# tylerrleee/mcmc-gpu

Hardware: AMD Instinct MI355X
Metric: chain-steps/sec on 256x256 grid x 1024 chains; accept-rate parity (higher is better)
Workload: dtype f64; 1 GPU; largeScaleChain 256x256 grid, 1024 chains/GPU, fp64, Philox spectral (Matern 0.9125) proposals, blocks 50-80, sigma_mc 5 (BASELINE configs[1]); chains_total=1024, mh_steps_per_bench_step=2048

## Files before the change

mcmc_gpu_amd/csrc/chain_strip_kernel.hip:

```cpp
#include "gsm_internal.h"
#include "device_util.h"
#include "proposal_device.h"
#include "strip_step.h"
#include <math.h>
#include <stdlib.h>
#include <algorithm>
#include <type_traits>

namespace gsm {

using namespace dev;
using strip::kST;
using strip::kSW;
using strip::kNR;

constexpr int kSUPW = 32 / kSW;
constexpr int kSMAXT = 16 / kSW;

static int strip_tile_len(const BlockTable& B) { return (B.max_bh + 2) * (B.max_bw + 2); }
static int strip_main_len(const FusedArgs& a) { return std::max(a.P.lds_main, strip_tile_len(a.T.B)); }
constexpr int kStripAux = 16 + 32 + 16 + kMathTabDoubles + 4 * kT1S + kMask1D;
size_t fused_strip_lds_doubles(const FusedArgs& a) { return (size_t)strip_main_len(a) + kStripAux; }

bool strip_table_ok(const StaticFields& S, const BlockTable& B, int lds_main, int tiles1_max, int tiles2_max) {
  static int on = -1;
  if (on < 0) { const char* v = getenv("GSM_STRIP"); on = v ? atoi(v) : 1; }
  const size_t lds = ((size_t)std::max(lds_main, strip_tile_len(B)) + kStripAux) * sizeof(double);
  return on && S.sA != nullptr && (uint64_t)S.H * S.W * 48u <= (4ull << 20) && B.n_sizes <= 64 && strip::table_ok(B.max_bh, B.max_bw) &&
         B.max_bh <= kT1S && B.max_bw <= kT1S && (B.masks == nullptr || B.mask1d != nullptr) && lds <= 80 * 1024 && 2 * tiles1_max <= kSW * kSUPW && tiles2_max <= kSW * kSMAXT;
}

using step::crec_t;
using step::load_c;

template <typename TS, bool FAST_DIV, bool NOISE>
__global__ __launch_bounds__(kST, 4) void chain_strip_kernel(const FusedArgs fa) {
  typedef step::cptr_t<FusedArgs> cargs_t;
  auto kargs = [] { return step::kargs<FusedArgs>(); };
  extern __shared__ double lds[];
  double* __restrict__ red = lds + fa.work_len;
  double* __restrict__ red2 = red + 16;
  double* __restrict__ carry = red2 + 32;
  double* __restrict__ mtab = red2 + 32 + 16;
  double* __restrict__ t1 = mtab + kMathTabDoubles;
  double* __restrict__ m1 = t1 + 4 * kT1S;

  const int tid = threadIdx.x;
  const int lane = tid & 63;
  const int wave = __builtin_amdgcn_readfirstlane(tid >> 6);
  const int chain = blockIdx.x;
  const int n_steps = fa.T.n_steps;
  const int gH = fa.T.S.H, gW = fa.T.S.W;
  const TS* const p_bed = (const TS*)fa.T.beds + (size_t)chain * (size_t)gH * (size_t)gW;
  const TS* const p_en = (const TS*)fa.T.energy + (size_t)chain * (size_t)gH * (size_t)gW;
  const double2* const p_st = fa.T.S.sA;
  const double two_sigma2 = fa.T.S.two_sigma2, rcp_two_sigma2 = fa.T.S.rcp_two_sigma2;
  const uint32_t n_cells = (uint32_t)gH * (uint32_t)gW;
  const crec_t rec0 = (crec_t)(uintptr_t)(fa.P.scalars + (size_t)chain * fa.P.n_steps);
  const uint64_t seed = NOISE ? 0ull : fa.P.seeds[chain];
  for (int i = tid; i < kMathTabDoubles; i += kST) mtab[i] = fa.P.mathtab[i];
  if (tid < 16) red[tid] = 0.0;
  __syncthreads();

  if (tid == 0) {
    const double h0 = fa.T.loss_sum[2 * chain], l0 = fa.T.loss_sum[2 * chain + 1];
    carry[0] = h0; carry[1] = l0; carry[2] = (h0 + l0) / two_sigma2;
  }
  __syncthreads();
  step::Window prev = {};
  const int64_t noise0 = NOISE ? (int64_t)chain * fa.P.n_steps * fa.noise_stride : 0;
  auto prop_rec = [&](crec_t r) {
    PropScalars q;
    q.scale = r->scale; q.nug = r->nug; q.aa = r->aa; q.m_const = r->m_const; q.m_kappa = r->m_kappa;
    q.bh = r->bh; q.bw = r->bw; q.fy_off = r->fy_off; q.g_off = r->g_off; q.pad = r->pad; q.mask_off = r->mask_off;
    q.m_nc = r->m_nc; q.m_m1 = r->m_m1; q.m_bh = r->m_bh; q.m_bw = r->m_bw;
    return q;
  };

  for (int s = 0; s < n_steps; ++s) {
    int ptid = tid;
    asm volatile("" : "+v"(ptid));
    auto relaunder = [&] { asm volatile("" : "+v"(ptid)); };
    const crec_t rec = rec0 + s;
    const int s_row = rec->row, s_col = rec->col, s_bh = rec->bh, s_bw = rec->bw;

    {
      const cargs_t K = kargs();
      const double* __restrict__ g1 = K->P.tab1d;
      if (tid >= kST - kMask1D) m1[tid - (kST - kMask1D)] = K->P.B.mask1d[rec->si * kMask1D + tid - (kST - kMask1D)];
      if (tid < 2 * s_bh) t1[(tid < s_bh) ? tid : kT1S + tid - s_bh] = g1[rec->t1h_off + tid];
      else if (tid >= 256 && tid < 256 + 2 * s_bw) {
        const int i = ptid - 256;
        const double v = g1[rec->t1w_off + i];
        t1[2 * kT1S + ((i < s_bw) ? i : kT1S + i - s_bw)] = (i < s_bw) ? v : -v;
      }
    }
    {
      const cargs_t K = kargs();
      const ProposeArgs pa = load_c(&K->P);
      const PropScalars q = prop_rec(rec);
      const PropGeom pg = prop_geom(pa, q.bh, q.bw);
      NoiseIn nz{nullptr, nullptr, nullptr};
      if (NOISE) {
        const cargs_t F = K;
        const int64_t o = noise0 + (int64_t)s * F->noise_stride;
        nz.re = F->noise_re + o; nz.im = F->noise_im + o;
      }
      coef_items<kST, NOISE, true>(ptid, pa, q, pg, seed, pa.step0 + s, lds, nz, mtab, pa.parseval ? red2 + 16 : nullptr);
    }
    if (step::halo_touches(step::clip_window(gH, gW, s_row, s_col, s_bh, s_bw), prev)) asm volatile("s_waitcnt vmcnt(0)" ::: "memory");
    asm volatile("s_waitcnt lgkmcnt(0)\n\ts_barrier" ::: "memory");
    const double dc0 = lds[0];
    {
      v4f64 uc[kSUPW], us[kSUPW];
      {
        const cargs_t K = kargs();
        const ProposeArgs pa = load_c(&K->P);
        const PropScalars q = prop_rec(rec);
        dft_stage1<kSW, kSUPW, kTabLds1D>(wave, ptid & 63, pa, q, prop_geom(pa, q.bh, q.bw), lds, t1, uc, us);
      }
      asm volatile("s_waitcnt lgkmcnt(0)\n\ts_barrier" ::: "memory");
      {
        const cargs_t K = kargs();
        const ProposeArgs pa = load_c(&K->P);
        relaunder();
        dft_tt_write<kSW, kSUPW>(wave, ptid & 63, prop_geom(pa, s_bh, s_bw), lds, uc, us);
      }
    }
    asm volatile("s_waitcnt lgkmcnt(0)\n\ts_barrier" ::: "memory");
    {
      const cargs_t K = kargs();
      const ProposeArgs pa = load_c(&K->P);
      const PropScalars q = prop_rec(rec);
      const PropGeom pg = prop_geom(pa, q.bh, q.bw);
      const int bw = q.bw;
      v4f64 fe[kSMAXT], fo[kSMAXT];
      const double mreg[kSMAXT][8] = {};
      relaunder();
      const int ln = ptid & 63;
      dft_stage2<kSW, kSMAXT, kTabLds1D>(wave, ln, pa, q, pg, lds, t1 + 2 * kT1S, fe, fo);
      const double gain = standardise<kSW, kSMAXT>(wave, ln, q, pg, dc0, red2, fe, fo, pa.parseval ? red2 + 16 : nullptr);
      NoiseIn nz{nullptr, nullptr, nullptr};
      if (NOISE) {
        const cargs_t F = K;
        const double* nb = F->noise_nug;
        if (nb) nz.nug = nb + noise0 + (int64_t)s * F->noise_stride;
      }
      const bool with_nugget = NOISE ? (nz.nug != nullptr) : (pa.rf.nugget_max > 0.0);
      emit_field<kSW, kSMAXT, kMaskLds1D>(wave, ln, pa, q, pg, fe, fo, mreg, gain, with_nugget, lds, [bw](int y, int x) { return (y + 1) * (bw + 2) + x + 1; }, m1);
      if (with_nugget) {
        __syncthreads();
        relaunder();
        nugget_pass<kST, NOISE>(ptid, pa, q, pg, seed, pa.step0 + s, nz, lds, [bw](int y, int x) { return (y + 1) * (bw + 2) + x + 1; }, mtab);
      }
    }
    relaunder();
    const step::Window Gw = step::clip_window(gH, gW, s_row, s_col, s_bh, s_bw);
    const strip::Window G = strip::make_window(gH, gW, s_row, s_col, s_bh, s_bw);
    const strip::Cfg cfg = strip::config(G.wh, G.ww);
    const strip::Lane L = strip::lane_setup(ptid & 63, wave, cfg, G, gH, gW);
    const rsrc_t r_bed = make_rsrc(p_bed, n_cells * (uint32_t)sizeof(TS));
    const rsrc_t r_en = make_rsrc(p_en, n_cells * (uint32_t)sizeof(TS));
    const rsrc_t r_st = make_rsrc(p_st, 3u * n_cells * 16u);
    uint32_t upd_bits;
    double acc_old;
    bool guard;
    {
      double vb[kNR + 2], ve[kNR];
      double2 a2[strip::kNA];
      if (G.interior) strip::load_state<TS, true>(L, cfg.n, gW, r_bed, r_en, r_st, vb, ve, a2);
      else strip::load_state<TS, false>(L, cfg.n, gW, r_bed, r_en, r_st, vb, ve, a2);
      asm volatile("s_waitcnt lgkmcnt(0)\n\ts_barrier" ::: "memory");
      const int ts = s_bw + 2;
      auto field = [&](int jj, bool) { return lds[L.tidx + jj * ts]; };
      if (G.interior) strip::phase_a<TS, true>(L, cfg.n, gW, s_bw, r_st, field, lds, vb, ve, a2, upd_bits, acc_old, guard);
      else strip::phase_a<TS, false>(L, cfg.n, gW, s_bw, r_st, field, lds, vb, ve, a2, upd_bits, acc_old, guard);
    }
    asm volatile("s_waitcnt lgkmcnt(0)\n\ts_barrier" ::: "memory");
    double en[kNR], vn[kNR];
    {
      double acc_new;
      const cargs_t K = kargs();
      const step::StepConsts SC{K->T.S.res, K->T.S.rcp_res, K->T.S.two_res, K->T.S.rcp_two_res};
      if (G.interior) strip::phase_d<TS, FAST_DIV, true>(L, cfg.n, gW, s_bw, r_st, n_cells * 16u, SC, lds, en, acc_new);
      else strip::phase_d<TS, FAST_DIV, false>(L, cfg.n, gW, s_bw, r_st, n_cells * 16u, SC, lds, en, acc_new);
      double delta = acc_new - acc_old;
      if (guard) delta = INFINITY;
      const double w_delta = wave64_sum(delta);
      if (lane == 0) red[wave] = w_delta;
    }
    strip::read_candidate(L, cfg.n, s_bw, lds, vn);
    const double s_hi = carry[0], s_lo = carry[1];
    double loss_prev = carry[2];
    asm volatile("s_waitcnt lgkmcnt(0)\n\ts_barrier" ::: "memory");
    const double sd = strip::waves_sum(red, lane);
    double c_hi, c_lo, loss_next;
    const bool acc = step::decide<FAST_DIV>(sd, sd == INFINITY, s_hi, s_lo, two_sigma2, rcp_two_sigma2, loss_prev, rec->u, c_hi, c_lo, loss_next);
    if (acc) {
      if (G.interior) strip::commit<TS, true, false>(L, cfg.n, gW, r_bed, r_en, r_en, vn, en, upd_bits);
      else strip::commit<TS, false, false>(L, cfg.n, gW, r_bed, r_en, r_en, vn, en, upd_bits);
      loss_prev = loss_next;
      if (tid == 0) {
        double n_hi, n_lo;
        two_sum(c_hi, c_lo, n_hi, n_lo);
        carry[0] = n_hi; carry[1] = n_lo; carry[2] = loss_next;
      }
      prev = Gw;
    } else {
      prev = step::Window{};
    }
    if (tid == 0) {
      const cargs_t Ke = kargs();
      const StepArgs a = load_c(&Ke->T);
      step::write_record(a, step::record_index(a, chain, s), loss_prev, acc, s_row, s_col, s_bh, s_bw);
    }
  }
  if (tid == 0) {
    fa.T.loss_sum[2 * chain] = carry[0];
    fa.T.loss_sum[2 * chain + 1] = carry[1];
  }
}

template <typename TS, bool FAST_DIV>
__global__ __launch_bounds__(kST, 4) void step_strip_kernel(const StepArgs a) {
  extern __shared__ double tile[];
  __shared__ double red[16];
  __shared__ int tab[2 * 64];
  const StaticFields& S = a.S;
  const int tid = threadIdx.x;
  const int lane = tid & 63;
  const int wave = __builtin_amdgcn_readfirstlane(tid >> 6);
  const int chain = blockIdx.x;
  const int H = S.H, W = S.W;
  const uint32_t n_cells = (uint32_t)H * (uint32_t)W;
  const size_t plane = (size_t)H * W;
  const rsrc_t r_bed = make_rsrc((const TS*)a.beds + (size_t)chain * plane, n_cells * (uint32_t)sizeof(TS));
  const rsrc_t r_en = make_rsrc((const TS*)a.energy + (size_t)chain * plane, n_cells * (uint32_t)sizeof(TS));
  const rsrc_t r_rs = make_rsrc(a.resampled + (size_t)chain * plane, n_cells * 4u);
  const rsrc_t r_st = make_rsrc(S.sA, 3u * n_cells * 16u);
  const step::StepConsts SC{S.res, S.rcp_res, S.two_res, S.rcp_two_res};

  double s_hi = a.loss_sum[2 * chain], s_lo = a.loss_sum[2 * chain + 1];
  double loss_prev = (s_hi + s_lo) / S.two_sigma2;
  for (int i = tid; i < a.B.n_sizes; i += kST) { tab[2 * i] = a.B.bh[i]; tab[2 * i + 1] = a.B.bw[i]; }
  if (tid < 16) red[tid] = 0.0;
  const int64_t rin0 = (int64_t)chain * a.in_stride;
  step::ReplayRec nxt = step::read_replay(a, rin0);
  __syncthreads();

  for (int s = 0; s < a.n_steps; ++s) {
    const int64_t rin = rin0 + s;
    const int64_t rout = step::record_index(a, chain, s);
    const step::ReplayRec cur = nxt;
    const bool has_next = s + 1 < a.n_steps;
    if (has_next) nxt = step::read_replay(a, rin + 1);
    if (!step::replay_valid(a, cur)) {
      if (tid == 0) step::reject_record(a, rout, loss_prev, cur);
      continue;
    }
    const int bh = tab[2 * cur.si], bw = tab[2 * cur.si + 1];
    const rsrc_t r_f = make_rsrc(a.fields + rin * a.field_stride, (uint32_t)(bh * bw) * 8u);
    const step::Window Gw = step::clip_window(H, W, cur.row, cur.col, bh, bw);
    const strip::Window G = strip::make_window(H, W, cur.row, cur.col, bh, bw);
    const strip::Cfg cfg = strip::config(G.wh, G.ww);
    const strip::Lane L = strip::lane_setup(lane, wave, cfg, G, H, W);
    uint32_t upd_bits;
    double acc_old;
    bool guard;
    {
      double vb[kNR + 2], ve[kNR];
      double2 a2[strip::kNA];
      auto field = [&](int jj, bool in) { return ld_f64<2>(r_f, in ? (uint32_t)(L.fidx + jj * bw) * 8u : kOOB); };
      if (G.interior) {
        strip::load_state<TS, true>(L, cfg.n, W, r_bed, r_en, r_st, vb, ve, a2);
        strip::phase_a<TS, true>(L, cfg.n, W, bw, r_st, field, tile, vb, ve, a2, upd_bits, acc_old, guard);
      } else {
        strip::load_state<TS, false>(L, cfg.n, W, r_bed, r_en, r_st, vb, ve, a2);
        strip::phase_a<TS, false>(L, cfg.n, W, bw, r_st, field, tile, vb, ve, a2, upd_bits, acc_old, guard);
      }
    }
    asm volatile("s_waitcnt lgkmcnt(0)\n\ts_barrier" ::: "memory");
    double en[kNR], vn[kNR];
    {
      double acc_new;
      if (G.interior) strip::phase_d<TS, FAST_DIV, true>(L, cfg.n, W, bw, r_st, n_cells * 16u, SC, tile, en, acc_new);
      else strip::phase_d<TS, FAST_DIV, false>(L, cfg.n, W, bw, r_st, n_cells * 16u, SC, tile, en, acc_new);
      double delta = acc_new - acc_old;
      if (guard) delta = INFINITY;
      const double w_delta = wave64_sum(delta);
      if (lane == 0) red[wave] = w_delta;
    }
    strip::read_candidate(L, cfg.n, bw, tile, vn);
    asm volatile("s_waitcnt lgkmcnt(0)\n\ts_barrier" ::: "memory");
    const double sd = strip::waves_sum(red, lane);
    double c_hi, c_lo, loss_next;
    const bool acc = step::decide<FAST_DIV>(sd, sd == INFINITY, s_hi, s_lo, S.two_sigma2, S.rcp_two_sigma2, loss_prev, cur.u, c_hi, c_lo, loss_next);
    if (acc) {
      if (G.interior) strip::commit<TS, true, true>(L, cfg.n, W, r_bed, r_en, r_rs, vn, en, upd_bits);
      else strip::commit<TS, false, true>(L, cfg.n, W, r_bed, r_en, r_rs, vn, en, upd_bits);
      two_sum(c_hi, c_lo, s_hi, s_lo);
      loss_prev = loss_next;
    }
    if (tid == 0) step::write_record(a, rout, loss_prev, acc, cur.row, cur.col, bh, bw);
    if (acc && has_next && (unsigned)nxt.si < (unsigned)a.B.n_sizes) {
      if (step::halo_touches(step::clip_window(H, W, nxt.row, nxt.col, tab[2 * nxt.si], tab[2 * nxt.si + 1]), Gw)) asm volatile("s_waitcnt vmcnt(0)" ::: "memory");
    }
    asm volatile("s_waitcnt lgkmcnt(0)\n\ts_barrier" ::: "memory");
  }
  if (tid == 0) {
    a.loss_sum[2 * chain] = s_hi;
    a.loss_sum[2 * chain + 1] = s_lo;
  }
}

template <typename TS>
static hipError_t launch_step_strip_t(const StepArgs& a, hipStream_t st) {
  return launch_pair<step_strip_kernel<TS, true>, step_strip_kernel<TS, false>>(
      a.S.fast_div, 80 * 1024, dim3(a.n_chains), dim3(kST), (size_t)strip_tile_len(a.B) * sizeof(double), st, a);
}
hipError_t launch_step_strip(const StepArgs& a, hipStream_t st) {
  if (!a.strip) return hipErrorInvalidValue;
  return a.f32_state ? launch_step_strip_t<float>(a, st) : launch_step_strip_t<double>(a, st);
}

template <typename TS, bool NOISE>
static hipError_t launch_fused_strip_t(const FusedArgs& a, hipStream_t st) {
  return launch_pair<chain_strip_kernel<TS, true, NOISE>, chain_strip_kernel<TS, false, NOISE>>(
      a.T.S.fast_div, 80 * 1024, dim3(a.T.n_chains), dim3(kST), fused_strip_lds_doubles(a) * sizeof(double), st, a);
}

hipError_t launch_chain_strip(const FusedArgs& a_in, hipStream_t st) {
  if (!a_in.T.strip || a_in.P.tab_max <= 0) return hipErrorInvalidValue;
  FusedArgs a = a_in;
  a.work_len = strip_main_len(a);
  a.fld_len = 0;
  return a.T.f32_state ? launch_fused_strip_t<float, false>(a, st) : launch_fused_strip_t<double, false>(a, st);
}

hipError_t launch_chain_strip_noise(const FusedArgs& a_in, hipStream_t st) {
  if (!a_in.T.strip || a_in.P.tab_max <= 0 || !a_in.noise_re || !a_in.noise_im) return hipErrorInvalidValue;
  FusedArgs a = a_in;
  a.work_len = strip_main_len(a);
  a.fld_len = 0;
  return a.T.f32_state ? launch_fused_strip_t<float, true>(a, st) : launch_fused_strip_t<double, true>(a, st);
}

}
```

mcmc_gpu_amd/csrc/gsm_api.hip:

```cpp
#include "gsm_context.h"
#include "math_tables.h"
#include "normal_score.h"
#include <math.h>
#include <string.h>
#include <algorithm>

using namespace gsm;

static thread_local std::string g_create_err;

int gsm::fail(gsm_handle h, int code, const std::string& msg) {
  if (h) h->err = msg; else g_create_err = msg;
  return code;
}

extern "C" const char* gsm_last_error(gsm_handle h) { return h ? h->err.c_str() : g_create_err.c_str(); }

extern "C" int gsm_create(gsm_handle* out, int32_t H, int32_t W, int32_t n_chains, int32_t dtype, int32_t device) {
  if (!out) return fail(nullptr, GSM_E_ARG, "gsm_create: out is NULL");
  *out = nullptr;
  if (H < 3 || W < 3 || n_chains < 1) return fail(nullptr, GSM_E_ARG, "gsm_create: need H,W >= 3 and n_chains >= 1");
  if ((int64_t)H * W > (1LL << 30)) return fail(nullptr, GSM_E_ARG, "gsm_create: grid too large");
  if (dtype != 0 && dtype != 1) return fail(nullptr, GSM_E_UNSUPPORTED, "gsm_create: dtype must be 0 (fp64 state) or 1 (fp32 state)");
  int ndev = 0;
  hipError_t e = hipGetDeviceCount(&ndev);
  if (e != hipSuccess || ndev < 1)
    return fail(nullptr, GSM_E_HIP, std::string("gsm_create: no HIP device: ") + hipGetErrorString(e));
  if (device < 0 || device >= ndev) return fail(nullptr, GSM_E_ARG, "gsm_create: device index out of range");
  e = hipSetDevice(device);
  if (e != hipSuccess) return fail(nullptr, GSM_E_HIP, std::string("hipSetDevice: ") + hipGetErrorString(e));
  gsm_context* c = new gsm_context();
  c->H = H; c->W = W; c->n_chains = n_chains; c->device = device; c->f32_state = dtype;
  e = c->d_err.ensure(1);
  if (e == hipSuccess) e = hipMemset(c->d_err.get(), 0, sizeof(int32_t));
  if (e != hipSuccess) { delete c; return fail(nullptr, GSM_E_HIP, std::string("hipMalloc: ") + hipGetErrorString(e)); }
  *out = c;
  return GSM_OK;
}

extern "C" int gsm_destroy(gsm_handle h) {
  if (!h) return GSM_OK;
  hipSetDevice(h->device);
  delete h;
  return GSM_OK;
}

extern "C" int gsm_set_static(gsm_handle h, const double* surf, const double* velx, const double* vely,
                              const double* dhdt, const double* smb, const double* crf_weight,
                              const uint8_t* update_mask, const uint8_t* mc_mask, double resolution,
                              double sigma_mc, void* stream) {
  if (!h) return GSM_E_ARG;
  if (!surf || !velx || !vely || !dhdt || !smb || !update_mask || !mc_mask)
    return fail(h, GSM_E_ARG, "gsm_set_static: NULL field");
  if (!(resolution > 0.0) || !(sigma_mc > 0.0)) return fail(h, GSM_E_ARG, "gsm_set_static: resolution and sigma_mc must be > 0");
  hipStream_t st = (hipStream_t)stream;
  HIPCHK(h, hipSetDevice(h->device));
  const size_t n = (size_t)h->H * h->W;
  const double* src[6] = {surf, velx, vely, dhdt, smb, crf_weight};
  for (int i = 0; i < 6; ++i) {
    if (!src[i]) { h->d_static[i].reset(); continue; }
    HIPCHK(h, h->d_static[i].assign(src[i], n, st));
  }
  HIPCHK(h, h->d_upd.assign(update_mask, n, st));
  HIPCHK(h, h->d_mc.assign(mc_mask, n, st));
  StaticFields& S = h->S;
  S.surf = h->d_static[0].get(); S.velx = h->d_static[1].get(); S.vely = h->d_static[2].get();
  S.dhdt = h->d_static[3].get(); S.smb = h->d_static[4].get(); S.weight = h->d_static[5].get();
  S.upd = h->d_upd.get(); S.mc = h->d_mc.get();
  S.H = h->H; S.W = h->W;
  S.res = resolution;
  S.two_res = 2.0 * resolution;
  S.rcp_res = 1.0 / S.res;
  S.rcp_two_res = 1.0 / S.two_res;
  S.two_sigma2 = 2 * (sigma_mc * sigma_mc);
  S.rcp_two_sigma2 = 1.0 / S.two_sigma2;
  {
    auto divisor_ok = [](double d) {
      uint64_t bits;
      memcpy(&bits, &d, sizeof(bits));
      const bool all_ones = (bits & 0xFFFFFFFFFFFFFull) == 0xFFFFFFFFFFFFFull;
      return !all_ones && d > 1e-100 && d < 1e100;
    };
    S.fast_div = (divisor_ok(S.res) && divisor_ok(S.two_sigma2)) ? 1 : 0;
  }
  HIPCHK(h, h->d_svx.ensure(n));
  HIPCHK(h, h->d_svy.ensure(n));
  HIPCHK(h, h->d_ds.ensure(n));
  HIPCHK(h, h->d_sABC.ensure(3 * n));
  double2 *sA = h->d_sABC.get(), *sB = sA + n, *sC = sA + 2 * n;
  HIPCHK(h, launch_pack_static(S, h->d_svx.get(), h->d_svy.get(), h->d_ds.get(), st));
  HIPCHK(h, launch_pack_flux_static(S, sA, sB, sC, st));
  S.svx = h->d_svx.get(); S.svy = h->d_svy.get(); S.ds = h->d_ds.get();
  S.sA = sA; S.sB = sB; S.sC = sC;
  HIPCHK(h, hipStreamSynchronize(st));
  h->have_static = true;
  return GSM_OK;
}

extern "C" int gsm_set_blocks(gsm_handle h, int32_t n_sizes, const int32_t* bh, const int32_t* bw,
                              const double* edge_masks_packed, const int64_t* mask_offsets, void* stream) {
  if (!h) return GSM_E_ARG;
  if (n_sizes < 1 || !bh || !bw) return fail(h, GSM_E_ARG, "gsm_set_blocks: empty block table");
  if (n_sizes > 64) return fail(h, GSM_E_UNSUPPORTED, "gsm_set_blocks: at most 64 block sizes");
  hipStream_t st = (hipStream_t)stream;
  HIPCHK(h, hipSetDevice(h->device));
  int max_bh = 0, max_bw = 0, cap = 0;
  int64_t mask_total = 0;
  for (int i = 0; i < n_sizes; ++i) {
    if (bh[i] < 2 || bw[i] < 2 || (bh[i] & 1) || (bw[i] & 1))
      return fail(h, GSM_E_ARG, "gsm_set_blocks: block sizes must be even and >= 2 (RandField.get_block_sizes makes them even)");
    if (bh[i] > h->H || bw[i] > h->W)
      return fail(h, GSM_E_ARG, "gsm_set_blocks: block larger than the grid (the reference's slices mismatch there)");
    max_bh = std::max(max_bh, bh[i]);
    max_bw = std::max(max_bw, bw[i]);
    cap = std::max(cap, (bh[i] + 2) * (bw[i] + 2));
    if (mask_offsets) mask_total = std::max<int64_t>(mask_total, mask_offsets[i] + (int64_t)bh[i] * bw[i]);
  }
  if (step_lds_bytes(cap) > 160 * 1024)
    return fail(h, GSM_E_UNSUPPORTED, "gsm_set_blocks: (bh+2)*(bw+2) window does not fit the 160 KiB LDS tile");
  h->d_factors.reset();
  h->n_classes = 0;
  for (auto& c : h->chol) c = gsm_context::CholScratch();
  HIPCHK(h, h->d_bh.assign(bh, (size_t)n_sizes, st));
  HIPCHK(h, h->d_bw.assign(bw, (size_t)n_sizes, st));
  if (edge_masks_packed && mask_offsets) {
    HIPCHK(h, h->d_mask_off.assign(mask_offsets, (size_t)n_sizes, st));
    HIPCHK(h, h->d_masks.assign(edge_masks_packed, (size_t)mask_total, st));
    h->d_mask1d.reset();
    {
      std::vector<double> hm((size_t)mask_total);
      HIPCHK(h, hipMemcpyAsync(hm.data(), edge_masks_packed, sizeof(double) * (size_t)mask_total, hipMemcpyDefault, st));
      HIPCHK(h, hipStreamSynchronize(st));
      std::vector<double> t1((size_t)n_sizes * kMask1D, 0.0);
      bool one_d = true;
      for (int i = 0; i < n_sizes && one_d; ++i) {
        const double* m = hm.data() + mask_offsets[i];
        const int H = bh[i], W = bw[i];
        if ((std::min(H, W) - 1) / 2 >= kMask1D) { one_d = false; break; }
        std::vector<char> have(kMask1D, 0);
        for (int y = 0; y < H && one_d; ++y)
          for (int x = 0; x < W; ++x) {
            const int d = std::min(std::min(y, H - 1 - y), std::min(x, W - 1 - x));
            const double v = m[(size_t)y * W + x];
            double& t = t1[(size_t)i * kMask1D + d];
            if (!have[d]) { have[d] = 1; t = v; }
            else if (memcmp(&t, &v, sizeof(double)) != 0) { one_d = false; break; }
          }
      }
      if (one_d) HIPCHK(h, h->d_mask1d.assign(t1.data(), t1.size(), st));
      HIPCHK(h, hipStreamSynchronize(st));
    }
  } else {
    h->d_masks.reset();
    h->d_mask_off.reset();
    h->d_mask1d.reset();
  }
  const int max_len = std::max(max_bh, max_bw);
  std::vector<int32_t> fy_off(max_len + 1, -1), g_off(max_len + 1, -1);
  std::vector<double> tb;
  int krmax = 0, n1max = 0, m1max = 0, kcmax = 0, tiles_max = 0;
  h->prop_tiles1 = 0;
  for (int i = 0; i < n_sizes; ++i) {
    const int n = bh[i];
    const int nrow = n / 2 + 1;
    const int KR = (nrow + 3) & ~3, NR = (nrow + 15) & ~15, N1 = (n + 15) & ~15;
    krmax = std::max(krmax, KR); n1max = std::max(n1max, N1);
    if (fy_off[n] < 0) {
      fy_off[n] = (int32_t)tb.size();
      tb.resize(tb.size() + (size_t)2 * KR * NR, 0.0);
      double* FC = tb.data() + fy_off[n];
      double* FS = FC + (size_t)KR * NR;
      for (int ky = 0; ky < nrow; ++ky)
        for (int y = 0; y < nrow; ++y) {
          const double ang = 2.0 * M_PI * (double)(((int64_t)ky * y) % n) / (double)n;
          FC[ky * NR + y] = cos(ang);
          FS[ky * NR + y] = sin(ang);
        }
    }
    const int w = bw[i];
    const int ncol = w / 2 + 1, Kc = (ncol + 3) & ~3, M1 = (ncol + 15) & ~15;
    m1max = std::max(m1max, M1); kcmax = std::max(kcmax, Kc);
    tiles_max = std::max(tiles_max, (N1 / 16) * (M1 / 16));
    const int NRh = ((n / 2) / 2 + 16) & ~15;
    h->prop_tiles1 = std::max(h->prop_tiles1, 2 * (M1 / 16) * (NRh / 16));
    if (g_off[w] < 0) {
      g_off[w] = (int32_t)tb.size();
      tb.resize(tb.size() + (size_t)2 * Kc * M1, 0.0);
      double* GC = tb.data() + g_off[w];
      double* GS = GC + (size_t)Kc * M1;
      for (int k = 0; k < ncol; ++k) {
        const double ck = (k == 0 || k == w / 2) ? 1.0 : 2.0;
        for (int x = 0; x < ncol; ++x) {
          const double ang = 2.0 * M_PI * (double)(((int64_t)k * x) % w) / (double)w;
          GC[k * M1 + x] = ck * cos(ang);
          GS[k * M1 + x] = -ck * sin(ang);
        }
      }
    }
  }
  auto stride16mod32 = [](int v) { int s = v; while ((s & 31) != 16) ++s; return s; };
  h->lds_sx = stride16mod32(m1max);
  h->lds_st = stride16mod32(n1max);
  h->lds_x_half = (krmax * h->lds_sx + 127) & ~127;
  h->lds_tt = 2 * kcmax * h->lds_st;
  h->prop_tiles = tiles_max;
  h->tables_len = (int)tb.size();
  h->tab_max = 0;
  for (int i = 0; i < n_sizes; ++i) {
    const int nrow = bh[i] / 2 + 1, ncol = bw[i] / 2 + 1;
    h->tab_max = std::max(h->tab_max, 2 * ((nrow + 3) & ~3) * ((nrow + 15) & ~15));
    h->tab_max = std::max(h->tab_max, 2 * ((ncol + 3) & ~3) * ((ncol + 15) & ~15));
  }
  {
    std::vector<int32_t> k2_off((size_t)n_sizes);
    int32_t tot = 0;
    for (int i = 0; i < n_sizes; ++i) { k2_off[i] = tot; tot += (bh[i] / 2 + 1) * (bw[i] / 2 + 1); }
    HIPCHK(h, h->d_k2_off.assign(k2_off.data(), k2_off.size(), st));
    h->d_k2.reset();
    HIPCHK(h, h->d_k2.ensure((size_t)tot));
    h->k2_resolution = 0.0;
  }
  HIPCHK(h, h->d_tables.assign(tb.data(), tb.size(), st));
// ... 195 lines not shown
```

mcmc_gpu_amd/csrc/gsm_internal.h:

```cpp
#pragma once
#include <hip/hip_runtime.h>
#include <stdint.h>
#include <string>
#include <vector>
#include "../../include/gsm.h"

namespace gsm {

constexpr int kMaxDevices = 64;
inline bool attr_needed_on_this_device(bool (&flags)[kMaxDevices], int& dev) {
  dev = 0;
  if (hipGetDevice(&dev) != hipSuccess || dev < 0 || dev >= kMaxDevices) { dev = -1; return true; }
  return !flags[dev];
}
template <auto K0, auto K1, class... Args>
inline hipError_t launch_pair(bool first, int lds_cap, dim3 grid, dim3 block, size_t lds, hipStream_t st, const Args&... args) {
  static bool attr_set[kMaxDevices] = {};
  int attr_dev;
  if (attr_needed_on_this_device(attr_set, attr_dev)) {
    hipError_t e = hipFuncSetAttribute((const void*)K0, hipFuncAttributeMaxDynamicSharedMemorySize, lds_cap);
    if (e == hipSuccess) e = hipFuncSetAttribute((const void*)K1, hipFuncAttributeMaxDynamicSharedMemorySize, lds_cap);
    if (e != hipSuccess) return e;
    if (attr_dev >= 0) attr_set[attr_dev] = true;
  }
  if (first) hipLaunchKernelGGL(K0, grid, block, lds, st, args...);
  else hipLaunchKernelGGL(K1, grid, block, lds, st, args...);
  return hipGetLastError();
}

struct StaticFields {
  const double* surf;
  const double* velx;
  const double* vely;
  const double* dhdt;
  const double* smb;
  const double* weight;
  const uint8_t* upd;
  const uint8_t* mc;
  const double2* svx;
  const double2* svy;
  const double2* ds;
  const double2* sA;
  const double2* sB;
  const double2* sC;
  int H, W;
  double res;
  double two_res;
  double rcp_res;
  double rcp_two_res;
  int fast_div;
  double two_sigma2;
  double rcp_two_sigma2;
};

struct BlockTable {
  const int32_t* bh;
  const int32_t* bw;
  const double* masks;
  const int64_t* mask_off;
  const double* mask1d;
  int n_sizes;
  int max_bh, max_bw;
};

struct StepArgs {
  StaticFields S;
  BlockTable B;
  int n_chains, n_steps;
  int tile_cap;
  void* beds;
  void* energy;
  int f32_state;
  uint32_t* resampled;
  double* loss_sum;
  const int32_t* size_idx;
  const int32_t* centre;
  const double* u;
  const double* fields;
  int64_t field_stride;
  double* loss;
  uint8_t* accept;
  int32_t* blocks;
  int64_t rec_stride;
  int64_t rec_offset;
  int64_t in_stride;
  int32_t* err_flag;
  int strip;
};

struct PropScalars {
  double scale, nug, range_x, range_y, u;
  double aa, m_const, m_kappa;
  int32_t si, row, col, bh;
  int32_t bw, fy_off, g_off, pad;
  int64_t mask_off;
  uint32_t m_nc, m_m1, m_tw, reserved;
  uint32_t m_bh, m_bw;
  int32_t t1h_off, t1w_off;
};

struct ProposeArgs {
  BlockTable B;
  gsm_rf_params rf;
  int H, W;
  int n_chains, n_steps;
  int64_t step0;
  const uint64_t* seeds;
  const int32_t* centres;
  int n_centres;
  int32_t* size_idx;
  int32_t* centre;
  double* u;
  double* fields;
  int64_t field_stride;
  double* rf_scalars;
  const double* tables;
  int tables_len;
  int tab_max;
  const int32_t* fy_off;
  const int32_t* g_off;
  int lds_sx, lds_st;
  int lds_x_half;
  int lds_tt;
  const double* mathtab;
  int lds_main;
  int tiles1_max, tiles2_max;
  const double* tab1d;
  const int32_t* t1_off;
  const double* k2tab;
  const int32_t* k2_off;
  PropScalars* scalars;
  int parseval;
  int split2;
};

struct FusedArgs {
  StepArgs T;
  ProposeArgs P;
  int work_len, fld_len;
  const double* noise_re; const double* noise_im; const double* noise_nug;
  int64_t noise_stride;
};

struct CholArgs {
  int n_classes, n_groups;
  const double* const* factors;
  int* counts;
  int* rec_off;
  int* tile_off;
  int* work_off;
  int64_t* z_off;
  int* group_of;
  int* order;
  double* scale;
  double* zbuf;
};

struct PcgDrawArgs {
  int H, W, n_chains, n_steps, n_sizes;
  gsm_rf_params rf;
  const int32_t* bh; const int32_t* bw;
  uint64_t* rf_state;
  uint64_t* ch_state;
  const uint8_t* region_mask;
  const uint64_t* jump; const uint64_t* zig;
  int32_t* size_idx; int32_t* centre; double* u; double* rf_scalars;
  double* noise_re; double* noise_im; double* nugget;
  int64_t field_stride;
  int32_t* err;
};
hipError_t launch_pcg64_draw(const PcgDrawArgs& a, hipStream_t st);
constexpr int kPcgJumpWords = 4 * 512;
void pcg64_host_tables(uint64_t* jump_out, const uint64_t** zig_out);
struct SgsDrawArgs;
hipError_t launch_sgs_draw_pcg64(const SgsDrawArgs& a, uint64_t* states, const uint64_t* jump, const uint64_t* zig, hipStream_t st);

struct SgsCellHdr {
  int32_t n;
  int32_t op;
  double sdz;
  double var;
  double c1;
};
struct SgsArgs {
  int H, W, n_chains;
  double* grid;
  const double* zcond;
  const int32_t* win;
  const double* xs;
  const double* ys;
  const double* lag;
  int hw, mi, mj, num_points;
  int ktype;
  int defer;
  const double* gmean;
  double radius, sill;
  const int32_t* cell_off;
  const int32_t* cell_cnt;
// ... 176 lines not shown
```

mcmc_gpu_amd/csrc/strip_step.h:

```cpp
#pragma once
#include "gsm_internal.h"
#include "device_util.h"
#include "step_common.h"
#include <math.h>

namespace gsm {
namespace strip {

using namespace dev;

constexpr int kST = 512;
constexpr int kSW = kST / 64;
constexpr int kNR = 16;

struct Cfg { int cs, g, sr, n; };

__host__ __device__ inline int rows_per_strip(int wh, int sr) {
  switch (sr) {
    case 8: return (wh + 7) >> 3;
    case 6: return (int)(((uint32_t)(wh + 5) * 10923u) >> 16);
    case 5: return (int)(((uint32_t)(wh + 4) * 13108u) >> 16);
    case 4: return (wh + 3) >> 2;
    case 2: return (wh + 1) >> 1;
    default: return wh;
  }
}
__host__ __device__ inline Cfg config(int wh, int ww) {
  Cfg c;
  if (ww <= 62) { c.cs = 6; c.g = 1; c.sr = 8; }
  else if (ww <= 70) { c.cs = 4; c.g = 5; c.sr = 6; }
  else if (ww <= 90) { c.cs = 5; c.g = 3; c.sr = 5; }
  else if (ww <= 124) { c.cs = 6; c.g = 2; c.sr = 4; }
  else if (ww <= 248) { c.cs = 6; c.g = 4; c.sr = 2; }
  else { c.cs = 6; c.g = 8; c.sr = 1; }
  c.n = rows_per_strip(wh, c.sr);
  return c;
}
__host__ inline bool table_ok(int max_bh, int max_bw) {
  if (max_bw > 496) return false;
  for (int ww = 1; ww <= max_bw; ++ww) if (config(max_bh, ww).n > kNR) return false;
  return true;
}

__host__ __device__ __forceinline__ int small_div(int t, int d) {
  const uint64_t lo = 32769ull | (16385ull << 16) | (10923ull << 32) | (8193ull << 48);
  const uint64_t hi = 6554ull | (5462ull << 16) | (4682ull << 32) | (4097ull << 48);
  const uint32_t m = (uint32_t)(((d <= 4) ? lo : hi) >> (16 * ((d - 1) & 3))) & 0xFFFFu;
  return (int)(((uint32_t)t * m) >> 15);
}

struct Window {
  int r0, c0, wh, ww;
  int mr0, mc0;
  int bw;
  bool interior;
};
__host__ __device__ __forceinline__ Window make_window(int H, int W, int row, int col, int bh, int bw) {
  const step::Window w = step::clip_window(H, W, row, col, bh, bw);
  return Window{w.r0, w.c0, w.wh, w.ww, w.mr0, w.mc0, bw, step::interior(H, W, w)};
}

enum : uint32_t {
  kFValid = 1u,
  kFColIn = 2u,
  kFColOwn = 4u,
  kFTopIn = 8u,
  kFBelowIn = 16u,
  kFAtLeft = 32u, kFAtRight = 64u,
};
struct Lane {
  uint32_t cell0;
  int fidx;
  int tidx;
  int rows;
  uint32_t flags;
  int lo, hi;
  int jtop, jbot;
};
__host__ __device__ __forceinline__ Lane lane_setup(const int lane, const int wave, const Cfg& c, const Window& g, const int H, const int W) {
  Lane L;
  const int C = 1 << c.cs;
  const int sub = lane >> c.cs, l = lane & (C - 1);
  const int sidx = wave * (64 >> c.cs) + sub;
  const int kr = small_div(sidx, c.g), kc = sidx - kr * c.g;
  const int wc = kc * (C - 2) + l - 1;
  const int gc = g.c0 + wc;
  int rows = min(c.n, g.wh - kr * c.n);
  const bool valid = (kr < c.sr) && (rows > 0) && (wc <= g.ww) && (gc >= 0) && (gc < W);
  if (!valid) rows = -2;
  const bool colin = valid && (wc >= 0) && (wc < g.ww);
  const bool colown = colin && (l >= 1) && (l <= C - 2);
  const int wr0 = kr * c.n - 1;
  const int gr0 = g.r0 + wr0;
  L.rows = rows;
  L.flags = (valid ? kFValid : 0u) | (colin ? kFColIn : 0u) | (colown ? kFColOwn : 0u) | ((valid && kr > 0) ? kFTopIn : 0u) |
            ((valid && kr * c.n + rows < g.wh) ? kFBelowIn : 0u) | ((gc == 0) ? kFAtLeft : 0u) | ((gc == W - 1) ? kFAtRight : 0u);
  L.lo = max(0, -gr0);
  L.hi = valid ? min(rows + 1, H - 1 - gr0) : -1;
  L.jtop = -gr0; L.jbot = H - 1 - gr0;
  L.cell0 = (uint32_t)(gr0 * W + gc);
  L.fidx = (g.mr0 + wr0) * g.bw + g.mc0 + wc;
  L.tidx = (g.mr0 + wr0 + 1) * (g.bw + 2) + g.mc0 + wc + 1;
  return L;
}
__host__ __device__ __forceinline__ bool has(const Lane& L, const uint32_t f) { return (L.flags & f) != 0u; }

__device__ __forceinline__ Lane fresh(Lane L) {
  asm volatile("" : "+v"(L.rows), "+v"(L.flags), "+v"(L.lo), "+v"(L.hi));
  return L;
}
__device__ __forceinline__ int fresh_s(int W) { asm volatile("" : "+s"(W)); return W; }

template <typename TS> struct RowIO;
template <> struct RowIO<double> {
  static __device__ __forceinline__ double load(rsrc_t r, uint32_t off, uint32_t soff) {
    return __builtin_bit_cast(double, __builtin_amdgcn_raw_buffer_load_b64(r, (int)off, (int)soff, 2));
  }
  static __device__ __forceinline__ void store(rsrc_t r, uint32_t off, uint32_t soff, double v) {
    __builtin_amdgcn_raw_buffer_store_b64(__builtin_bit_cast(v2i32, v), r, (int)off, (int)soff, 2);
  }
};
template <> struct RowIO<float> {
  static __device__ __forceinline__ double load(rsrc_t r, uint32_t off, uint32_t soff) {
    return (double)__builtin_bit_cast(float, __builtin_amdgcn_raw_buffer_load_b32(r, (int)off, (int)soff, 2));
  }
  static __device__ __forceinline__ void store(rsrc_t r, uint32_t off, uint32_t soff, double v) {
    __builtin_amdgcn_raw_buffer_store_b32(__builtin_bit_cast(int, (float)v), r, (int)off, (int)soff, 2);
  }
};
__device__ __forceinline__ double ld_f64_s(rsrc_t r, uint32_t off, uint32_t soff) {
  return __builtin_bit_cast(double, __builtin_amdgcn_raw_buffer_load_b64(r, (int)off, (int)soff, 0));
}

template <bool INTERIOR>
__device__ __forceinline__ void row_offsets(const Lane& L, const int jj, const int W, const uint32_t cb, uint32_t& off, uint32_t& soff) {
  if (INTERIOR) { off = L.cell0 * cb; soff = (uint32_t)(jj * W) * cb; }
  else { off = (L.cell0 + (uint32_t)(jj * W)) * cb; soff = 0u; }
}
__host__ __device__ __forceinline__ bool row_exists(const Lane& L, const int jj) { return jj >= L.lo && jj <= L.hi; }
__host__ __device__ __forceinline__ bool row_own(const Lane& L, const int jj) { return (jj >= 1) && (jj <= kNR) && (jj <= L.rows); }
struct WriteMasks { bool w0, w1, w2; };
__host__ __device__ __forceinline__ WriteMasks write_masks(const Lane& L) {
  WriteMasks m;
  const bool valid = has(L, kFValid), colin = has(L, kFColIn);
  m.w0 = valid && !(has(L, kFTopIn) && colin);
  m.w1 = valid && (has(L, kFColOwn) || !colin);
  m.w2 = valid && !(has(L, kFBelowIn) && colin);
  return m;
}
template <bool INTERIOR>
__host__ __device__ __forceinline__ bool cell_written(const Lane& L, const WriteMasks& m, const int jj) {
  bool w = (jj == 0) ? m.w0 : ((jj <= L.rows && m.w1) || (jj - 1 == L.rows && m.w2));
  if (!INTERIOR) w = w && row_exists(L, jj);
  return w;
}

constexpr int kNA = 4;
template <typename TS, bool INTERIOR, int PARTS = 3>
__device__ __forceinline__ void load_state(const Lane& L_in, const int n, const int W_in, const rsrc_t r_bed, const rsrc_t r_en, const rsrc_t r_st,
                                           double (&vb)[kNR + 2], double (&ve)[kNR], double2 (&a2)[kNA]) {
  const Lane L = fresh(L_in);
  const int W = fresh_s(W_in);
  const WriteMasks wm = write_masks(L);
  const bool colown = has(L, kFColOwn);
  uint32_t oob = kOOB;
  asm volatile("" : "+v"(oob));
  const uint32_t ownS = colown ? L.cell0 * (uint32_t)sizeof(TS) : oob, own16 = colown ? L.cell0 * 16u : oob;
#pragma unroll
  for (int jj = 0; jj < kNR + 2; ++jj) {
    if (PARTS & 1) vb[jj] = 0.0;
    if ((PARTS & 2) && jj >= 1 && jj <= kNR) ve[jj - 1] = 0.0;
    if ((PARTS & 2) && jj >= 1 && jj <= kNA) a2[jj - 1] = make_double2(0.0, 0.0);
    if (jj <= n + 1) {
      uint32_t off, soff, off16, soff16;
      row_offsets<INTERIOR>(L, jj, W, (uint32_t)sizeof(TS), off, soff);
      row_offsets<INTERIOR>(L, jj, W, 16u, off16, soff16);
      if (PARTS & 1) vb[jj] = RowIO<TS>::load(r_bed, cell_written<INTERIOR>(L, wm, jj) ? off : oob, soff);
      if ((PARTS & 2) && jj >= 1 && jj <= kNR) {
        const bool ro = row_own(L, jj);
        if (jj <= kNA) a2[jj - 1] = ld_f64x2(r_st, ro ? (INTERIOR ? own16 : (colown ? off16 : oob)) : oob, soff16);
        ve[jj - 1] = RowIO<TS>::load(r_en, ro ? (INTERIOR ? ownS : (colown ? off : oob)) : oob, soff);
      }
    }
  }
}

template <typename TS, bool INTERIOR, class Field>
__device__ __forceinline__ void phase_a(const Lane& L_in, const int n, const int W_in, const int bw, const rsrc_t r_st, Field field,
                                        double* __restrict__ tile, double (&vb)[kNR + 2], double (&ve)[kNR], double2 (&a2)[kNA],
                                        uint32_t& upd_bits, double& acc_old, bool& guard) {
  constexpr bool F32 = sizeof(TS) == 4;
  const Lane L = fresh(L_in);
  const int W = fresh_s(W_in);
  const WriteMasks wm = write_masks(L);
  const bool colown = has(L, kFColOwn);
  uint32_t oob = kOOB;
  asm volatile("" : "+v"(oob));
  const uint32_t own16 = colown ? L.cell0 * 16u : oob;
  guard = false;
  upd_bits = 0u;
  const int ts = bw + 2;
#pragma unroll
  for (int jj = 0; jj < kNR + 2; ++jj) {
    if (jj <= n + 1) {
      double v = vb[jj];
      if (jj >= 1 && jj <= kNR) {
        const bool own = row_own(L, jj) && colown;
        const double2 A2 = a2[(jj - 1) % kNA];
        if (jj + kNA <= kNR && jj + kNA <= n) {
          uint32_t off, soff;
          row_offsets<INTERIOR>(L, jj + kNA, W, 16u, off, soff);
          a2[(jj - 1) % kNA] = ld_f64x2(r_st, row_own(L, jj + kNA) ? (INTERIOR ? own16 : (colown ? off : oob)) : oob, soff);
// ... 140 lines not shown
```

Before: 16.95 million chain-steps/s.

## Clip strip windows to the update-mask bounding box to skip inactive cells

Setup now copies the update mask to the host and computes the bounding box of updatable cells, padded by one for the halo, and stores it in StaticFields. Both the fused and replay strip kernels intersect each block window with this box, so lanes no longer load, evaluate or commit cells that can never change. The replay path also forces the window fields to be wave-uniform with readfirstlane and recomputes the halo-check window only when it is needed, to reduce register pressure. The clipped window shifts the mask offsets, and a window of zero area is marked as empty. This relies on the loss contributions outside the box being unchanged and adds a host sync at setup.

```diff
diff --git a/mcmc_gpu_amd/csrc/chain_strip_kernel.hip b/mcmc_gpu_amd/csrc/chain_strip_kernel.hip
--- a/mcmc_gpu_amd/csrc/chain_strip_kernel.hip
+++ b/mcmc_gpu_amd/csrc/chain_strip_kernel.hip
@@ -156,7 +156,11 @@
     }
     relaunder();
     const step::Window Gw = step::clip_window(gH, gW, s_row, s_col, s_bh, s_bw);
-    const strip::Window G = strip::make_window(gH, gW, s_row, s_col, s_bh, s_bw);
+    strip::Window G;
+    {
+      const cargs_t K = kargs();
+      G = strip::make_window(gH, gW, s_row, s_col, s_bh, s_bw, K->T.S.tr0, K->T.S.tr1, K->T.S.tc0, K->T.S.tc1);
+    }
     const strip::Cfg cfg = strip::config(G.wh, G.ww);
     const strip::Lane L = strip::lane_setup(ptid & 63, wave, cfg, G, gH, gW);
     const rsrc_t r_bed = make_rsrc(p_bed, n_cells * (uint32_t)sizeof(TS));
@@ -260,8 +264,11 @@
     }
     const int bh = tab[2 * cur.si], bw = tab[2 * cur.si + 1];
     const rsrc_t r_f = make_rsrc(a.fields + rin * a.field_stride, (uint32_t)(bh * bw) * 8u);
-    const step::Window Gw = step::clip_window(H, W, cur.row, cur.col, bh, bw);
-    const strip::Window G = strip::make_window(H, W, cur.row, cur.col, bh, bw);
+    strip::Window G;
+    {
+      const step::cptr_t<StepArgs> K = step::kargs<StepArgs>();
+      G = strip::uniform(strip::make_window(H, W, cur.row, cur.col, bh, bw, K->S.tr0, K->S.tr1, K->S.tc0, K->S.tc1));
+    }
     const strip::Cfg cfg = strip::config(G.wh, G.ww);
     const strip::Lane L = strip::lane_setup(lane, wave, cfg, G, H, W);
     uint32_t upd_bits;
@@ -303,6 +310,9 @@
     }
     if (tid == 0) step::write_record(a, rout, loss_prev, acc, cur.row, cur.col, bh, bw);
     if (acc && has_next && (unsigned)nxt.si < (unsigned)a.B.n_sizes) {
+      int w_row = cur.row;
+      asm volatile("" : "+s"(w_row));
+      const step::Window Gw = step::clip_window(H, W, w_row, cur.col, bh, bw);
       if (step::halo_touches(step::clip_window(H, W, nxt.row, nxt.col, tab[2 * nxt.si], tab[2 * nxt.si + 1]), Gw)) asm volatile("s_waitcnt vmcnt(0)" ::: "memory");
     }
     asm volatile("s_waitcnt lgkmcnt(0)\n\ts_barrier" ::: "memory");
diff --git a/mcmc_gpu_amd/csrc/gsm_api.hip b/mcmc_gpu_amd/csrc/gsm_api.hip
--- a/mcmc_gpu_amd/csrc/gsm_api.hip
+++ b/mcmc_gpu_amd/csrc/gsm_api.hip
@@ -68,6 +68,22 @@
   S.dhdt = h->d_static[3].get(); S.smb = h->d_static[4].get(); S.weight = h->d_static[5].get();
   S.upd = h->d_upd.get(); S.mc = h->d_mc.get();
   S.H = h->H; S.W = h->W;
+  {
+    std::vector<uint8_t> um(n);
+    HIPCHK(h, hipMemcpyAsync(um.data(), update_mask, n, hipMemcpyDefault, st));
+    HIPCHK(h, hipStreamSynchronize(st));
+    int r_lo = h->H, r_hi = -1, c_lo = h->W, c_hi = -1;
+    for (int r = 0; r < h->H; ++r) {
+      const uint8_t* m = um.data() + (size_t)r * h->W;
+      for (int c = 0; c < h->W; ++c)
+        if (m[c]) { r_lo = std::min(r_lo, r); r_hi = r; c_lo = std::min(c_lo, c); c_hi = std::max(c_hi, c); }
+    }
+    if (r_hi < 0) S.tr0 = S.tr1 = S.tc0 = S.tc1 = 0;
+    else {
+      S.tr0 = std::max(r_lo - 1, 0); S.tr1 = std::min(r_hi + 2, h->H);
+      S.tc0 = std::max(c_lo - 1, 0); S.tc1 = std::min(c_hi + 2, h->W);
+    }
+  }
   S.res = resolution;
   S.two_res = 2.0 * resolution;
   S.rcp_res = 1.0 / S.res;
diff --git a/mcmc_gpu_amd/csrc/gsm_internal.h b/mcmc_gpu_amd/csrc/gsm_internal.h
--- a/mcmc_gpu_amd/csrc/gsm_internal.h
+++ b/mcmc_gpu_amd/csrc/gsm_internal.h
@@ -44,6 +44,7 @@
   const double2* sB;
   const double2* sC;
   int H, W;
+  int32_t tr0, tr1, tc0, tc1;
   double res;
   double two_res;
   double rcp_res;
diff --git a/mcmc_gpu_amd/csrc/strip_step.h b/mcmc_gpu_amd/csrc/strip_step.h
--- a/mcmc_gpu_amd/csrc/strip_step.h
+++ b/mcmc_gpu_amd/csrc/strip_step.h
@@ -58,6 +58,22 @@
 __host__ __device__ __forceinline__ Window make_window(int H, int W, int row, int col, int bh, int bw) {
   const step::Window w = step::clip_window(H, W, row, col, bh, bw);
   return Window{w.r0, w.c0, w.wh, w.ww, w.mr0, w.mc0, bw, step::interior(H, W, w)};
+}
+__host__ __device__ __forceinline__ Window make_window(int H, int W, int row, int col, int bh, int bw, int tr0, int tr1, int tc0, int tc1) {
+  const step::Window w = step::clip_window(H, W, row, col, bh, bw);
+  step::Window t = w;
+  t.r0 = max(w.r0, tr0); t.r1 = min(w.r1, tr1);
+  t.c0 = max(w.c0, tc0); t.c1 = min(w.c1, tc1);
+  if (t.r1 <= t.r0 || t.c1 <= t.c0) return Window{w.r0, w.c0, 0, 0, w.mr0, w.mc0, bw, false};
+  return Window{t.r0, t.c0, t.r1 - t.r0, t.c1 - t.c0, w.mr0 + (t.r0 - w.r0), w.mc0 + (t.c0 - w.c0), bw, step::interior(H, W, t)};
+}
+
+__device__ __forceinline__ Window uniform(Window g) {
+  g.r0 = __builtin_amdgcn_readfirstlane(g.r0); g.c0 = __builtin_amdgcn_readfirstlane(g.c0);
+  g.wh = __builtin_amdgcn_readfirstlane(g.wh); g.ww = __builtin_amdgcn_readfirstlane(g.ww);
+  g.mr0 = __builtin_amdgcn_readfirstlane(g.mr0); g.mc0 = __builtin_amdgcn_readfirstlane(g.mc0);
+  g.interior = __builtin_amdgcn_readfirstlane((int)g.interior) != 0;
+  return g;
 }
 
 enum : uint32_t {
```

After: 17.81 million chain-steps/s (median of 6 runs). 1.05x the previous value.
